# WindowsXp-Beta/nos

Hardware: AMD Instinct MI355X
Metric: aggregate GPU util % + schedulable fractional pods/node at 1/2/4/8 MI355X (higher is better)
Workload: dtype fp32

## Files before the change

### csrc/hip/gemm_f32h.hip

```cpp
#include <stdlib.h>

#include <type_traits>

#include "attn_d64_planes.h"
#include "common.h"
#include "epilogue.h"
#include "lds_pipe.h"
#include "split_f16.h"

namespace {

using nos::gelu_erf;
using nos::glds16;
using nos::wait_stages;

template <int E>
using EpiC = std::integral_constant<int, E>;

struct Batch {
  int nb = 1;
  long long a = 0, rinv = 0, w = 0, csc = 0, c = 0, r = 0, bias = 0;
};

constexpr int BK = 32;

__device__ __forceinline__ int swz(int row) { return (row >> 2) & 3; }

using nos::kvp::KvOut;

struct PlaneOut {
  unsigned short* p = nullptr;
  long long pplane = 0;
  int ldp = 0;
  float sc = 1.f;
};

struct LnIo {
  const float* x = nullptr;
  const float2* sin = nullptr;
  float2* sout = nullptr;
  int ldx = 0, nparts = 0, pw = 0, spart = 0;
  float eps = 0.f, sc = 1.f;
};

__device__ __forceinline__ void chan_merge(float& n, float& mean, float& m2, float nb, float mb, float m2b) {
  const float tot = n + nb;
  if (!(nb > 0.f)) return;
  const float d = mb - mean, f = nb / tot;
  mean = fmaf(d, f, mean);
  m2 += m2b + d * d * n * f;
  n = tot;
}

template <int BM, int BN, int WGM, int WGN, bool PERSIST, int RS = 2, int MODE = 0, bool BATCHED = false>
__global__ __launch_bounds__(64 * WGM * WGN, 2) void gemm_h3_kernel(
    const _Float16* __restrict__ Ap, int lda, long long aplane, const float* __restrict__ rinv, float rconst,
    const _Float16* __restrict__ Wp, int ldw, long long wplane, const float* __restrict__ csc,
    const float* __restrict__ bias, const float* __restrict__ R, int ldr0, float* __restrict__ C, int ldc0, int M,
    int N, int K, int epi, int tiles_m, int tiles_n, KvOut kv, PlaneOut po, Batch bt, LnIo ln) {
  constexpr int NW = WGM * WGN, MI = BM / (32 * WGM), NI = BN / (32 * WGN);
  static_assert(NW == 4 && MI >= 1 && NI >= 1, "4 waves");
  constexpr int ROWB = BK * 2, CH = ROWB / 16, RPP = 1024 / ROWB;
  static_assert(RS == 2 || RS == 3, "ring depth");
  constexpr int TA = 2 * BM * ROWB, STAGE = TA + 2 * BN * ROWB;
  constexpr int APW = TA / 1024 / NW, WPW = 2 * BN * ROWB / 1024 / NW;
  static_assert(APW * NW * 1024 == TA && WPW * NW * 1024 == 2 * BN * ROWB, "equal DMA count per wave");
  constexpr int LPS = APW + WPW;
  static_assert((RS - 2) * LPS < 64, "vmcnt range");
  static_assert(MODE == 0 || (BM == 128 && !BATCHED && (BN == 128 || BN == 64) && (RS == 2 || (MODE == 2 && RS == 3))),
                "the LayerNorm hand-off runs 128 x 128 or 128 x 64 tiles (the producer also on a 3-deep ring)");
  static_assert(MODE != 2 || BM * BN * 4 <= RS * STAGE, "the statistics tile fits the ring");
  extern __shared__ __attribute__((aligned(16))) unsigned char smem[];

  const int tid = threadIdx.x, wid = __builtin_amdgcn_readfirstlane(tid >> 6), lane = tid & 63;
  const int c0 = lane & 31, h0 = lane >> 5;
  const int wm = wid / WGN, wn = wid % WGN;
  const bool wide = (epi & EPI_WIDE) != 0;
  epi &= ~EPI_WIDE;
  const int ntiles1 = tiles_m * tiles_n, ntiles = BATCHED ? ntiles1 * bt.nb : ntiles1;
  const int nk = K / BK;
  nos::XcdChunk chunk;
  if constexpr (PERSIST) {
    chunk = nos::xcd_chunk(blockIdx.x, gridDim.x, ntiles);
  } else {
    chunk.first = nos::xcd_remap(blockIdx.x, ntiles);
    chunk.end = chunk.first + 1;
    chunk.step = 1;
  }
  for (int tt = chunk.first; tt < chunk.end; tt += chunk.step) {
    if (PERSIST && tt != chunk.first) __syncthreads();
    const int bb = BATCHED ? tt / ntiles1 : 0, t1 = BATCHED ? tt - bb * ntiles1 : tt;
    const int tm = t1 / tiles_n, tn = t1 - tm * tiles_n;
    const int m0 = tm * BM, n0 = tn * BN;
    const _Float16* __restrict__ Ab = BATCHED ? Ap + bb * bt.a : Ap;
    const _Float16* __restrict__ Wb = BATCHED ? Wp + bb * bt.w : Wp;
    const float* __restrict__ rinvb = BATCHED && rinv != nullptr ? rinv + bb * bt.rinv : rinv;
    const float* __restrict__ cscb = BATCHED ? csc + bb * bt.csc : csc;
    float* __restrict__ Cb = BATCHED && C != nullptr ? C + bb * bt.c : C;
    const float* __restrict__ Rb = BATCHED && R != nullptr ? R + bb * bt.r : R;
    const float* __restrict__ biasb = BATCHED && bias != nullptr ? bias + bb * bt.bias : bias;

    auto stage_a = [&](int k0, unsigned char* dst) {
#pragma unroll
      for (int i = 0; i < APW; ++i) {
        const int p = wid * APW + i;
        const int plane = p / (BM / RPP), rb = (p % (BM / RPP)) * RPP;
        const int row = rb + lane / CH;
        int g = m0 + row;
        g = g < M ? g : M - 1;
        glds16(Ab + plane * aplane + (long long)g * lda + k0 + (((lane % CH) ^ swz(row)) << 3),
               dst + plane * BM * ROWB + rb * ROWB);
      }
    };
    auto stage_w = [&](int k0, unsigned char* dst) {
#pragma unroll
      for (int i = 0; i < WPW; ++i) {
        const int p = wid * WPW + i;
        const int plane = p / (BN / RPP), rb = (p % (BN / RPP)) * RPP;
        const int row = rb + lane / CH;
        int g = n0 + row;
        g = g < N ? g : N - 1;
        glds16(Wb + plane * wplane + (long long)g * ldw + k0 + (((lane % CH) ^ swz(row)) << 3),
               dst + TA + plane * BN * ROWB + rb * ROWB);
      }
    };
    auto stage = [&](int k0, unsigned char* dst) {
      stage_a(k0, dst);
      stage_w(k0, dst);
    };

    f32x16_t acc[MI][NI];
#pragma unroll
    for (int i = 0; i < MI; ++i)
#pragma unroll
      for (int j = 0; j < NI; ++j)
#pragma unroll
        for (int r = 0; r < 16; ++r) acc[i][j][r] = 0.f;

    struct Frag {
      f16x8_t a[MI][2], w[NI][2];
    };
    auto load = [&](const unsigned char* base, int s, Frag& f) {
#pragma unroll
      for (int i = 0; i < MI; ++i) {
        const int row = wm * (BM / WGM) + i * 32 + c0;
#pragma unroll
        for (int p = 0; p < 2; ++p)
          f.a[i][p] = *reinterpret_cast<const f16x8_t*>(base + p * BM * ROWB + row * ROWB +
                                                        (((2 * s + h0) ^ swz(row)) << 4));
      }
#pragma unroll
      for (int j = 0; j < NI; ++j) {
        const int row = wn * (BN / WGN) + j * 32 + c0;
#pragma unroll
        for (int p = 0; p < 2; ++p)
          f.w[j][p] = *reinterpret_cast<const f16x8_t*>(base + TA + p * BN * ROWB + row * ROWB +
                                                        (((2 * s + h0) ^ swz(row)) << 4));
      }
    };
    auto mma = [&](const Frag& f) {
#pragma unroll
      for (int i = 0; i < MI; ++i)
#pragma unroll
        for (int j = 0; j < NI; ++j) acc[i][j] = nos::mma3h(f.a[i], f.w[j], acc[i][j]);
    };

    if constexpr (MODE == 1) {
    constexpr int AR = BM * 4 / (64 * NW);
    constexpr int RSTEP = 64 * NW / 4;
    const int q = tid & 3;
    float mul[AR], add[AR];
    const float* xr[AR];
#pragma unroll
    for (int i = 0; i < AR; ++i) {
      int g = m0 + (tid >> 2) + RSTEP * i;
      g = g < M ? g : M - 1;
      xr[i] = ln.x + (long long)g * ln.ldx + q * 8;
      const float2* st = ln.sin + (long long)g * ln.nparts;
      float n = 0.f, mean = 0.f, m2 = 0.f;
      for (int p = 0; p < ln.nparts; ++p) {
        const float2 v = st[p];
        const int nb = min(ln.pw, K - p * ln.pw);
        chan_merge(n, mean, m2, (float)nb, v.x, v.y);
      }
      mul[i] = rsqrtf(m2 / (float)K + ln.eps) * ln.sc;
      add[i] = -mean * mul[i];
    }
    float4 xa[AR][2];
    auto aload = [&](int k0) {
#pragma unroll
      for (int i = 0; i < AR; ++i) {
        xa[i][0] = *reinterpret_cast<const float4*>(xr[i] + k0);
        xa[i][1] = *reinterpret_cast<const float4*>(xr[i] + k0 + 4);
      }
    };
    auto awrite = [&](unsigned char* dst) {
#pragma unroll
      for (int i = 0; i < AR; ++i) {
        const int row = (tid >> 2) + RSTEP * i;
        const float4 u = xa[i][0], w = xa[i][1];
        f16x2_t h0, l0, h1, l1, h2, l2, h3, l3;
        nos::split2h(f32x2_t{fmaf(u.x, mul[i], add[i]), fmaf(u.y, mul[i], add[i])}, h0, l0);
        nos::split2h(f32x2_t{fmaf(u.z, mul[i], add[i]), fmaf(u.w, mul[i], add[i])}, h1, l1);
        nos::split2h(f32x2_t{fmaf(w.x, mul[i], add[i]), fmaf(w.y, mul[i], add[i])}, h2, l2);
        nos::split2h(f32x2_t{fmaf(w.z, mul[i], add[i]), fmaf(w.w, mul[i], add[i])}, h3, l3);
        const int off = row * ROWB + ((q ^ swz(row)) << 4);
        *reinterpret_cast<f16x8_t*>(dst + off) = f16x8_t{h0.x, h0.y, h1.x, h1.y, h2.x, h2.y, h3.x, h3.y};
        *reinterpret_cast<f16x8_t*>(dst + BM * ROWB + off) = f16x8_t{l0.x, l0.y, l1.x, l1.y, l2.x, l2.y, l3.x, l3.y};
      }
    };
    aload(0);
    stage_w(0, smem);
    asm volatile("s_waitcnt vmcnt(0)" ::: "memory");
    awrite(smem);
    if (nk > 1) {
      aload(BK);
      stage_w(BK, smem + STAGE);
    }
    asm volatile("s_waitcnt lgkmcnt(0)" ::: "memory");
    __builtin_amdgcn_s_barrier();
    Frag fa, fb;
    load(smem, 0, fa);
    for (int kt = 0; kt < nk; ++kt) {
      const unsigned char* cur = smem + (kt & 1) * STAGE;
      load(cur, 1, fb);
      mma(fa);
      __builtin_amdgcn_sched_barrier(0);
      if (kt + 1 < nk) {
        asm volatile("s_waitcnt vmcnt(0)" ::: "memory");
        awrite(smem + ((kt + 1) & 1) * STAGE);
      }
      __builtin_amdgcn_sched_barrier(0);
      mma(fb);
      __builtin_amdgcn_sched_barrier(0);
      if (kt + 1 < nk) {
        asm volatile("s_waitcnt lgkmcnt(0)" ::: "memory");
        __builtin_amdgcn_s_barrier();
        if (kt + 2 < nk) {
          aload((kt + 2) * BK);
          stage_w((kt + 2) * BK, smem + (kt & 1) * STAGE);
        }
        load(smem + ((kt + 1) & 1) * STAGE, 0, fa);
      }
      __builtin_amdgcn_sched_barrier(0);
    }
    } else if constexpr (RS == 2) {
    stage(0, smem);
    if (nk > 1) stage(BK, smem + STAGE);
    if (nk > 1) {
      asm volatile("s_waitcnt vmcnt(%0)" ::"n"(LPS) : "memory");
    } else {
      asm volatile("s_waitcnt vmcnt(0)" ::: "memory");
    }
    __builtin_amdgcn_s_barrier();
    Frag fa, fb;
    load(smem, 0, fa);
    for (int kt = 0; kt < nk; ++kt) {
      const unsigned char* cur = smem + (kt & 1) * STAGE;
      load(cur, 1, fb);
      mma(fa);
      __builtin_amdgcn_sched_barrier(0);
      if (kt + 1 < nk) {
        asm volatile("s_waitcnt vmcnt(0)" ::: "memory");
        asm volatile("s_waitcnt lgkmcnt(0)" ::: "memory");
        __builtin_amdgcn_s_barrier();
        if (kt + 2 < nk) stage((kt + 2) * BK, smem + (kt & 1) * STAGE);
        load(smem + ((kt + 1) & 1) * STAGE, 0, fa);
      }
      mma(fb);
      __builtin_amdgcn_sched_barrier(0);
    }
    } else {
#pragma unroll
    for (int q = 0; q < RS - 1; ++q)
      if (q < nk) stage(q * BK, smem + q * STAGE);
    for (int kt = 0; kt < nk; ++kt) {
      wait_stages<LPS>(min(RS - 2, nk - 1 - kt));
      asm volatile("s_waitcnt lgkmcnt(0)" ::: "memory");
      __builtin_amdgcn_s_barrier();
      if (kt + RS - 1 < nk) stage((kt + RS - 1) * BK, smem + ((kt + RS - 1) % RS) * STAGE);
      const unsigned char* cur = smem + (kt % RS) * STAGE;
      Frag f0, f1;
      load(cur, 0, f0);
      load(cur, 1, f1);
      mma(f0);
      mma(f1);
    }
    }
    __syncthreads();

    int c = c0, h = h0, ldc = ldc0, ldr = ldr0;
    asm volatile("" : "+v"(c), "+v"(h));
    asm volatile("" : "+s"(ldc), "+s"(ldr));
    float rsv[MI][16], rbv[MI][16];
    if (rinvb != nullptr) {
#pragma unroll
      for (int i = 0; i < MI; ++i)
#pragma unroll
        for (int r = 0; r < 16; ++r) {
          const int m = m0 + wm * (BM / WGM) + i * 32 + (r & 3) + 8 * (r >> 2) + 4 * h;
          rsv[i][r] = rinvb[m < M ? m : M - 1];
        }
    } else {
#pragma unroll
      for (int i = 0; i < MI; ++i)
#pragma unroll
        for (int r = 0; r < 16; ++r) rsv[i][r] = rconst;
    }
#pragma unroll
    for (int i = 0; i < MI; ++i)
#pragma unroll
      for (int r = 0; r < 16; ++r) {
        const int m = m0 + wm * (BM / WGM) + i * 32 + (r & 3) + 8 * (r >> 2) + 4 * h;
        rbv[i][r] = (BATCHED && (epi & EPI_BIAS_ROW)) ? biasb[m < M ? m : M - 1] : 0.f;
      }
    auto epilogue = [&](auto ec) -> bool {
      constexpr int E = decltype(ec)::value;
      auto has = [&](int f) -> bool {
        if constexpr (E < 0) return (epi & f) != 0;
        else return (E & f) != 0;
      };
      if constexpr (MODE == 2) {
// ... 146 lines not shown
              const int rl = wm * (BM / WGM) + i * 32 + (r & 3) + 8 * (r >> 2) + 4 * h;
              float v = fmaf(acc[i][j][r], rsv[i][r] * cs, p2 + rbv[i][r]);
              if (BATCHED && has(EPI_RESID_PRE)) v += Rt[(unsigned)(rl * ldr + cl)];
              if (has(EPI_GELU)) v = gelu_erf(v);
              if (has(EPI_RELU)) v = fmaxf(v, 0.f);
              if (has(EPI_RESID)) v += Rt[(unsigned)(rl * ldr + cl)];
              Ct[(unsigned)(rl * ldc + cl)] = v;
            }
          }
        }
        return true;
      }
      return false;
    };
    bool done = false;
    if constexpr (MODE == 1) {
      if (epi == EPI_BIAS) done = epilogue(EpiC<EPI_BIAS>{});
      else if (epi == (EPI_BIAS | EPI_GELU)) done = epilogue(EpiC<EPI_BIAS | EPI_GELU>{});
      else done = epilogue(EpiC<-1>{});
    } else if constexpr (MODE == 2) {
      if (epi == (EPI_BIAS | EPI_RESID)) done = epilogue(EpiC<EPI_BIAS | EPI_RESID>{});
      else if (epi == EPI_BIAS) done = epilogue(EpiC<EPI_BIAS>{});
      else done = epilogue(EpiC<-1>{});
    } else if constexpr (BATCHED) {
      done = epilogue(EpiC<-1>{});
    } else {
      switch (epi) {
        case EPI_BIAS: done = epilogue(EpiC<EPI_BIAS>{}); break;
        case EPI_BIAS | EPI_GELU: done = epilogue(EpiC<EPI_BIAS | EPI_GELU>{}); break;
        case EPI_BIAS | EPI_RESID: done = epilogue(EpiC<EPI_BIAS | EPI_RESID>{}); break;
        default: done = epilogue(EpiC<-1>{}); break;
      }
    }
    if (done) continue;
#pragma unroll
    for (int j = 0; j < NI; ++j) {
      const int n = n0 + wn * (BN / WGN) + j * 32 + c;
      const int nc = n < N ? n : N - 1;
      const float cs = cscb[nc];
      const float p2 = (epi & EPI_BIAS) ? biasb[nc] : 0.f;
#pragma unroll
      for (int i = 0; i < MI; ++i) {
#pragma unroll
        for (int r = 0; r < 16; ++r) {
          const int m = m0 + wm * (BM / WGM) + i * 32 + (r & 3) + 8 * (r >> 2) + 4 * h;
          float v = fmaf(acc[i][j][r], rsv[i][r] * cs, p2 + rbv[i][r]);
          if (BATCHED && (epi & EPI_RESID_PRE) && m < M && n < N) v += Rb[(long long)m * ldr + n];
          if ((epi & EPI_GELU)) v = gelu_erf(v);
          if ((epi & EPI_RELU)) v = fmaxf(v, 0.f);
          if (m < M && n < N) {
            if ((epi & EPI_RESID)) v += Rb[(long long)m * ldr + n];
            if (kv.kvs != nullptr && n >= kv.qcols) {
              const int t = (n - kv.qcols) >= kv.hd;
              const int col = n - kv.qcols - t * kv.hd;
              const int b = kv.S == M ? 0 : m / kv.S;
              const long long row = (long long)b * kv.skvp + (m - b * kv.S);
              const float x = v * kv.kvsc[t * (kv.hd >> 6) + (col >> 6)];
              const _Float16 h0 = (_Float16)x;
              const _Float16 h1 = (_Float16)(x - (float)h0);
              unsigned short* dst = kv.kvs + (row * nos::kvp::H3 + nos::kvp::H3 / 2 * t) * kv.hd + col;
              dst[0] = __builtin_bit_cast(unsigned short, h0);
              dst[kv.hd] = __builtin_bit_cast(unsigned short, h1);
            } else if (po.p != nullptr) {
              const float x = v * po.sc;
              const _Float16 h0 = (_Float16)x;
              const _Float16 h1 = (_Float16)(x - (float)h0);
              po.p[(long long)m * po.ldp + n] = __builtin_bit_cast(unsigned short, h0);
              po.p[po.pplane + (long long)m * po.ldp + n] = __builtin_bit_cast(unsigned short, h1);
            } else {
              Cb[(long long)m * ldc + n] = v;
            }
          }
        }
      }
    }
  }
}

bool g_wide_planes = [] {
  const char* e = getenv("NOS_AMD_H3_WIDE_PLANES");
  return e == nullptr || atoi(e) != 0;
}();

bool wide_planes_ok(const KvOut& kv, const PlaneOut& po) {
  if (!g_wide_planes) return false;
  if (po.p != nullptr)
    return !(((uintptr_t)po.p) & 15) && !(po.ldp % 8) && !(po.pplane % 8);
  if (kv.kvs != nullptr) return !(((uintptr_t)kv.kvs) & 15) && !(kv.hd % 8) && !(kv.qcols % 8);
  return false;
}

struct H3Call {
  const _Float16* a = nullptr;
  int lda = 0;
  long long aplane = 0;
  const float* rinv = nullptr;
  float rconst = 0.f;
  const _Float16* w = nullptr;
  int ldw = 0;
  long long wplane = 0;
  const float* csc = nullptr;
  const float* bias = nullptr;
  const float* R = nullptr;
  int ldr = 0;
  float* C = nullptr;
  int ldc = 0;
  int M = 0, N = 0, K = 0, epi = 0;
  KvOut kv;
  PlaneOut po;
  Batch bt;
  LnIo ln;
};

template <int BM, int BN, int WGM, int WGN, int RS = 2, bool BATCHED = false, int MODE = 0>
int launch_t(const H3Call& c, hipStream_t st) {
  const int tiles_m = (c.M + BM - 1) / BM, tiles_n = (c.N + BN - 1) / BN;
  const long long ntiles = (long long)tiles_m * tiles_n * c.bt.nb;
  if (ntiles > (1LL << 30)) return (int)hipErrorInvalidValue;
  const size_t lds = RS * (size_t)(2 * BM * BK * 2 + 2 * BN * BK * 2);
  constexpr int NT = 64 * WGM * WGN;
  const int epi = !BATCHED && wide_planes_ok(c.kv, c.po) ? c.epi | EPI_WIDE : c.epi;
  auto* plain = gemm_h3_kernel<BM, BN, WGM, WGN, false, RS, MODE, BATCHED>;
  decltype(plain) persistent = nullptr;
  if constexpr (!BATCHED) persistent = gemm_h3_kernel<BM, BN, WGM, WGN, true, RS, MODE, BATCHED>;
  return nos::launch_items(persistent, plain, NT, lds, ntiles, st, c.a, c.lda, c.aplane, c.rinv, c.rconst, c.w, c.ldw,
                           c.wplane, c.csc, c.bias, c.R, c.ldr, c.C, c.ldc, c.M, c.N, c.K, epi, tiles_m, tiles_n, c.kv,
                           c.po, c.bt, c.ln);
}

bool g_lds_epi = true;
int g_hot_ring = 2;
int g_hot_bn = 128;

template <int F4, int LPR = 64>
__global__ __launch_bounds__(256) void split_rows_h3_kernel(const float* __restrict__ A, int lda,
                                                            _Float16* __restrict__ P, int ldp, long long pplane,
                                                            float* __restrict__ rinv, int M, int K, int ln,
                                                            float eps, int eln) {
  typedef __attribute__((ext_vector_type(4))) _Float16 f16x4_t;
  constexpr int RPB = 256 / LPR;
  const int row = blockIdx.x * RPB + (int)(threadIdx.x / LPR);
  const int lane = threadIdx.x % LPR;
  if (row >= M) return;
  const float* a = A + (long long)row * lda;
  constexpr int NR = F4 > 0 ? F4 : 1;
  float4 v[NR];
  auto get = [&](int i, int k) -> float4 {
    if constexpr (F4 > 0) return v[i];
    return *reinterpret_cast<const float4*>(a + k);
  };
  const int nchunk = F4 > 0 ? F4 : (K + 4 * LPR - 1) / (4 * LPR);
  if constexpr (F4 > 0) {
#pragma unroll
    for (int i = 0; i < F4; ++i) {
// ... 151 lines not shown
  for (int o = 16; o > 0; o >>= 1) q += __shfl_xor(q, o, 64);
  if (lane == 0) out[row] = float2{mu, q};
}

}

NOS_API int nos_row_stats(const float* X, int ldx, void* stats, int M, int K, hipStream_t stream) {
  if (M <= 0 || K <= 0 || (K % 4) || (ldx % 4) || ldx < K || !X || !stats || (((uintptr_t)X) & 15) ||
      (((uintptr_t)stats) & 7))
    return (int)hipErrorInvalidValue;
  hipLaunchKernelGGL(row_stats_kernel, dim3((unsigned)((M + 7) / 8)), dim3(256), 0, stream, X, ldx,
                     static_cast<float2*>(stats), M, K);
  return (int)hipGetLastError();
}

NOS_API int nos_gemm_f32h3_set_lds_epilogue(int on) {
  g_lds_epi = on != 0;
  return 0;
}

NOS_API int nos_gemm_f32h3_set_hot_bn(int bn) {
  if (bn != 128 && bn != 64) return (int)hipErrorInvalidValue;
  g_hot_bn = bn;
  return 0;
}

NOS_API int nos_gemm_f32h3_hot_bn() { return g_hot_bn; }

NOS_API int nos_gemm_f32h3_set_hot_ring(int rs) {
  if (rs != 2 && rs != 3) return (int)hipErrorInvalidValue;
  g_hot_ring = rs;
  return 0;
}

NOS_API int nos_split_rows_h3(const float* A, int lda, void* P, int ldp, long long pplane, float* rinv, int M, int K,
                              int ln, float eps, int eln, hipStream_t stream) {
  if (M <= 0 || K <= 0 || (K % 4) || (lda % 4) || (ldp % 4) || ldp < K || pplane < (long long)M * ldp)
    return (int)hipErrorInvalidValue;
  if ((((uintptr_t)A) | ((uintptr_t)P)) & 15) return (int)hipErrorInvalidValue;
  if (eln < -126 || eln > 126 || ln < 0 || ln > 2) return (int)hipErrorInvalidValue;
  auto* p = static_cast<_Float16*>(P);
  const dim3 grid((unsigned)((M + 3) / 4)), blk(256);
  if (K <= 512) {
    const dim3 g2((unsigned)((M + 7) / 8));
    hipLaunchKernelGGL((split_rows_h3_kernel<4, 32>), g2, blk, 0, stream, A, lda, p, ldp, pplane, rinv, M, K, ln, eps,
                       eln);
  } else if (K <= 1024)
    hipLaunchKernelGGL(split_rows_h3_kernel<4>, grid, blk, 0, stream, A, lda, p, ldp, pplane, rinv, M, K, ln, eps, eln);
  else if (K <= 2048)
    hipLaunchKernelGGL(split_rows_h3_kernel<8>, grid, blk, 0, stream, A, lda, p, ldp, pplane, rinv, M, K, ln, eps, eln);
  else if (K <= 4096)
    hipLaunchKernelGGL(split_rows_h3_kernel<16>, grid, blk, 0, stream, A, lda, p, ldp, pplane, rinv, M, K, ln, eps,
                       eln);
  else
    hipLaunchKernelGGL(split_rows_h3_kernel<0>, grid, blk, 0, stream, A, lda, p, ldp, pplane, rinv, M, K, ln, eps, eln);
  return (int)hipGetLastError();
}

NOS_API int nos_split_cols_h3(const float* X, int ldx, long long bsx, int M, int K, int nb, void* P, int ldp,
                              long long pplane, float* rinv, float* work, hipStream_t stream) {
  const int Mp = (M + 31) / 32 * 32;
  if (M <= 0 || K <= 0 || nb <= 0 || ldx < K || (nb > 1 && bsx < (long long)(M - 1) * ldx + K) || ldp < Mp ||
      (ldp % 8) || pplane < (long long)nb * K * ldp || !X || !P || !rinv || !work || nb > 65535 ||
      (long long)(M + 63) / 64 > 65535)
    return (int)hipErrorInvalidValue;
  if ((((uintptr_t)P) & 15) || (pplane % 8)) return (int)hipErrorInvalidValue;
// ... 165 lines not shown
```

### csrc/hip/lds_pipe.h

```cpp
#pragma once
#include "common.h"

namespace nos {

__device__ __forceinline__ void glds16(const void* g, unsigned char* lds_wave_base) {
  const unsigned lds = __builtin_amdgcn_readfirstlane(
      (unsigned)(uintptr_t)(__attribute__((address_space(3))) unsigned char*)lds_wave_base);
  asm volatile("s_nop 0\n\tglobal_load_lds_dwordx4 %0, off" ::"v"(g), "{m0}"(lds) : "memory");
}

__device__ __forceinline__ void glds16_s(const void* sbase, unsigned voff, unsigned char* lds_wave_base) {
  const unsigned lds = __builtin_amdgcn_readfirstlane(
      (unsigned)(uintptr_t)(__attribute__((address_space(3))) unsigned char*)lds_wave_base);
  asm volatile("s_nop 0\n\tglobal_load_lds_dwordx4 %0, %1" ::"v"(voff), "s"(sbase), "{m0}"(lds) : "memory");
}

__device__ __forceinline__ void glds16_builtin(const void* g, unsigned char* lds_wave_base) {
  __builtin_amdgcn_global_load_lds(g, (__attribute__((address_space(3))) void*)lds_wave_base, 16, 0, 0);
}

__device__ __forceinline__ void dma_wait_publish() {
  asm volatile("s_waitcnt vmcnt(0)" ::: "memory");
  __syncthreads();
}

template <int LPS>
__device__ __forceinline__ void wait_stages(int n) {
  if (n <= 0)
    asm volatile("s_waitcnt vmcnt(0)" ::: "memory");
  else if (n == 1)
    asm volatile("s_waitcnt vmcnt(%0)" ::"n"(LPS) : "memory");
  else if (n == 2)
    asm volatile("s_waitcnt vmcnt(%0)" ::"n"(2 * LPS) : "memory");
  else
    asm volatile("s_waitcnt vmcnt(%0)" ::"n"(3 * LPS) : "memory");
}

}
```

### nos_amd/models/pod.py

```python
from __future__ import annotations

import argparse
import json
import os
import sys
import time
from pathlib import Path
from typing import Callable

import numpy as np

STATE_STARTING, STATE_READY, STATE_FAILED, STATE_DONE = 0.0, 1.0, 2.0, 3.0
_COLS = 4


class StatusBoard:

    def __init__(self, path: str | os.PathLike, pods: int | None = None):
        self.path = Path(path)
        if pods is not None:
            np.zeros((1 + pods, _COLS), dtype=np.float64).tofile(self.path)
        self.arr = np.memmap(self.path, dtype=np.float64, mode="r+")
        self.arr = self.arr.reshape(-1, _COLS)

# ... 34 lines not shown
    elif dtype == "bf16":
        from ..ops import _lib

        _lib.require_native_on_gpu()
        m = YolosDetector(cfg, backend="native")
        tdt = torch.bfloat16
    else:
        raise ValueError(f"dtype {dtype!r}")
    m.reset_parameters(seed)
    m = m.to(device, tdt).eval()
    x = make_demo_input(cfg, device=device, dtype=tdt, hw=hw if device == "cuda" else cfg.image_size, seed=seed)
    return m, x


def _die_with_parent() -> Callable[[], bool]:
    ppid0 = os.getppid()
    try:
        import ctypes
        import signal

        ctypes.CDLL(None, use_errno=True).prctl(1, int(signal.SIGTERM), 0, 0, 0)
    except Exception:
        pass
    return lambda: os.getppid() != ppid0


def kernel_config(memory_fraction: float | None, env: dict | None = None, cu_budget: int = 0) -> dict[str, str]:
    env = os.environ if env is None else env
    whole = memory_fraction is None or memory_fraction >= 0.99
    if cu_budget and not whole:
        gf = "latency"
    else:
        gf = "latency" if whole else "small"
    return {"gemm_bf16": env.get("NOS_AMD_GEMM_POLICY") or ("latency" if whole else "throughput"),
            "gemm_f32": env.get("NOS_AMD_GEMM_F32_POLICY") or gf,
            "attention_f32": env.get("NOS_AMD_ATTN_F32_VARIANT") or ("h3" if whole else "h3n"),
            "f32_math": env.get("NOS_AMD_F32_MATH") or "h3",
            "gemm_f32x6_tile": env.get("NOS_AMD_X6_TILE") or ("policy" if whole else "128x128"),
            "ln_handoff": env.get("NOS_AMD_LN_HANDOFF") or "on",
            "h3_epilogue": env.get("NOS_AMD_H3_EPILOGUE") or "lds",
            "h3_hot_ring": env.get("NOS_AMD_H3_HOT_RING") or "2",
            "h3_hot_bn": env.get("NOS_AMD_H3_HOT_BN") or "128"}


def slice_cu_budget(env: dict | None = None) -> int:
    env = os.environ if env is None else env
    if env.get("NOS_AMD_CU_BUDGET") is not None:
        return int(env["NOS_AMD_CU_BUDGET"])
    m = env.get("ROC_GLOBAL_CU_MASK")
    if not m:
        return 0
    try:
        return bin(int(m, 16)).count("1")
    except ValueError:
        return 0


class _ServerTenant:

    def __init__(self, client, keep_outputs: bool = False):
        self.client, self.keep_outputs, self.outputs = client, keep_outputs, ()

    def launch(self) -> None:
        if self.keep_outputs:
            self.outputs = self.client.infer(outputs=True)[0]
        else:
            self.client.infer()
# ... 172 lines not shown
```

### nos_amd/ops/__init__.py

```python
from __future__ import annotations

import math
from typing import NamedTuple

import torch
import torch.nn.functional as F

from . import _lib

EPI_BIAS, EPI_GELU, EPI_RESID, EPI_RELU = 1, 2, 4, 8


def _stream() -> int:
    return torch.cuda.current_stream().cuda_stream


def _ptr(t: torch.Tensor | None) -> int | None:
    return None if t is None else t.data_ptr()


def linear_ref(x, weight, bias=None, act=None, residual=None):
    y = x.float() @ weight.float().t()
    if bias is not None:
        y = y + bias.float()
# ... 330 lines not shown
def h3_planes_active(attention: bool = False) -> bool:
    return _F32_MATH == "h3" and (not attention or _ATTN_F32_VARIANT.startswith("h3"))


def set_f32_math(mode: str) -> None:
    global _F32_MATH
    if mode not in ("exact", "x6", "h3"):
        raise ValueError(f"f32 math must be 'exact', 'x6' or 'h3', got {mode!r}")
    _F32_MATH = mode


def f32_math() -> str:
    return _F32_MATH


def set_gemm_f32x6_tile(tile: str) -> None:
    names = {"policy": -1, "128x64": 3, "128x128": 5, "wide": 6, "256x128": 7}
    code = names[tile] if tile in names else int(tile)
    _lib.check(_lib.lib().nos_gemm_f32x6_set_tile(code), "nos_gemm_f32x6_set_tile")


def set_gemm_f32h3_lds_epilogue(on: bool) -> None:
    _lib.check(_lib.lib().nos_gemm_f32h3_set_lds_epilogue(int(bool(on))), "nos_gemm_f32h3_set_lds_epilogue")


def set_gemm_f32h3_hot_ring(stages: int) -> None:
    _lib.check(_lib.lib().nos_gemm_f32h3_set_hot_ring(int(stages)), "nos_gemm_f32h3_set_hot_ring")


def set_gemm_f32h3_hot_bn(bn: int) -> None:
    _lib.check(_lib.lib().nos_gemm_f32h3_set_hot_bn(int(bn)), "nos_gemm_f32h3_set_hot_bn")


def stats_pw() -> int:
    return int(_lib.lib().nos_gemm_f32h3_hot_bn())


def set_gemm_f32x6_pipeline(on: bool) -> None:
    _lib.check(_lib.lib().nos_gemm_f32x6_set_pipeline(int(bool(on))), "nos_gemm_f32x6_set_pipeline")


def split_bf16x3(t: torch.Tensor) -> torch.Tensor:
    t = t.float()
    p0 = t.to(torch.bfloat16)
    r = t - p0.float()
    p1 = r.to(torch.bfloat16)
    p2 = (r - p1.float()).to(torch.bfloat16)
    return torch.stack([p0, p1, p2]).contiguous()


@torch.no_grad()
def split_f32_weight(w: torch.Tensor) -> torch.Tensor:
    key = id(w)
    hit = _SPLIT_CACHE.get(key)
    if hit is not None:
        ref, ver, ptr, planes = hit
        if ref() is w and ver == w._version and ptr == w.data_ptr():
            return planes
    import weakref

    planes = split_bf16x3(w)
    _SPLIT_CACHE[key] = (weakref.ref(w, lambda _r, k=key: _SPLIT_CACHE.pop(k, None)), w._version, w.data_ptr(),
                         planes)
    return planes


# ... 20 lines not shown


def set_attention_f32_variant(variant: str) -> None:
    global _ATTN_F32_VARIANT
    x6 = {"x6": 0, "x6n": 1, "x6k1": 1, "x6k2": 2, "x6k3": 3, "x6k4": 4,
          "h3": 0, "h3n": 1, "h3k1": 1, "h3k2": 2, "h3k3": 3, "h3k4": 4}
    code = {"auto": 0, "w4k64": 1, "w4k64g2": 2, "w4k32": 3, "w2k64": 4, "w8k64": 5, "w4k32o4": 6,
            "w4k32g2": 7}.get(variant, 0)
    if variant not in x6 and code == 0 and variant != "auto":
        raise KeyError(variant)
    _lib.check(_lib.lib().nos_attn_f32_set_variant(code), "nos_attn_f32_set_variant")
    if variant in x6:
        _lib.check(_lib.lib().nos_attn_f32x6_set_kvsplit(x6[variant]), "nos_attn_f32x6_set_kvsplit")
    _ATTN_F32_VARIANT = variant


_ATTN_F32_VARIANT = "auto"


def attention_f32_variant() -> str:
    return _ATTN_F32_VARIANT


def apply_kernel_config(cfg: dict) -> None:
    set_gemm_policy(cfg["gemm_bf16"])
    set_gemm_f32_policy(cfg["gemm_f32"])
    set_attention_f32_variant(cfg["attention_f32"])
    set_f32_math(cfg["f32_math"])
    set_gemm_f32x6_tile(cfg["gemm_f32x6_tile"])
    set_ln_handoff(cfg.get("ln_handoff", "on") == "on")
    set_gemm_f32h3_lds_epilogue(cfg.get("h3_epilogue", "lds") == "lds")
    set_gemm_f32h3_hot_ring(int(cfg.get("h3_hot_ring", "2")))
    set_gemm_f32h3_hot_bn(int(cfg.get("h3_hot_bn", "128")))


@torch.no_grad()
def fold_layernorm(weight: torch.Tensor, bias: torch.Tensor | None, gamma: torch.Tensor, beta: torch.Tensor
                   ) -> tuple[torch.Tensor, torch.Tensor, torch.Tensor]:
    wg = (weight.float() * gamma.float()[None, :]).to(weight.dtype).contiguous()
    c1 = wg.float().sum(dim=1).contiguous()
    c2 = (weight.float() * beta.float()[None, :]).sum(dim=1)
    if bias is not None:
        c2 = c2 + bias.float()
    return wg, c1, c2.contiguous()


def linear_ln_ref(x, wg, c1, c2, act=None, eps=1e-12):
    xf = x.float()
    mu = xf.mean(-1, keepdim=True)
    var = xf.var(-1, unbiased=False, keepdim=True)
    y = ((xf @ wg.float().t()) - mu * c1) * torch.rsqrt(var + eps) + c2
    if act == "gelu":
        y = F.gelu(y)
    elif act == "relu":
        y = F.relu(y)
    return y.to(x.dtype)


def linear_ln(x: torch.Tensor, wg: torch.Tensor, c1: torch.Tensor, c2: torch.Tensor, act: str | None = None,
              eps: float = 1e-12, out: torch.Tensor | None = None, max_wg: int = 0,
              pre=None) -> torch.Tensor:
    if not x.is_cuda:
        return linear_ln_ref(x, wg, c1, c2, act, eps)
    K = x.shape[-1]
    N = wg.shape[0]
    x2 = x.reshape(-1, K)
# ... 294 lines not shown
```

### nos_amd/ops/_lib.py

```python
from __future__ import annotations

import ctypes
import os
import threading
from pathlib import Path

_LIB_PATH = Path(os.environ.get("NOS_AMD_HIP_LIB") or
                 Path(__file__).resolve().parent.parent / "_native" / "libnos_hip.so")
_lock = threading.Lock()
_lib: ctypes.CDLL | None = None
_err: str | None = None

c_int, c_ll, c_float, c_void_p, c_double = (ctypes.c_int, ctypes.c_longlong, ctypes.c_float,
                                            ctypes.c_void_p, ctypes.c_double)

_SIGS = {
    "nos_attn_fwd_d64": [c_void_p, c_void_p, c_void_p, c_void_p, c_int, c_int, c_int, c_int, c_int,
                         c_ll, c_int, c_ll, c_float, c_void_p],
    "nos_attn_fwd_f32_d64": [c_void_p, c_void_p, c_void_p, c_void_p, c_int, c_int, c_int, c_int, c_int,
                             c_ll, c_int, c_ll, c_float, c_void_p],
    "nos_attn_fwd_f32x6_d64": [c_void_p, c_void_p, c_void_p, c_void_p, c_int, c_int, c_int, c_int, c_int,
                               c_ll, c_int, c_ll, c_float, c_void_p, c_ll, c_void_p],
    "nos_attn_f32x6_workspace": [c_int, c_int, c_int, c_int],
    "nos_attn_fwd_f32x6_presplit_d64": [c_void_p, c_void_p, c_int, c_int, c_int, c_int, c_int, c_ll, c_int, c_ll,
# ... 111 lines not shown
                 c_int, c_int, c_int, c_float, c_void_p],
    "nos_gemv_partials": [c_void_p, c_ll, c_int, c_int, c_int, c_int, c_int, c_int, c_void_p, c_int, c_int, c_void_p,
                          c_void_p, c_int, c_void_p, c_int, c_int, c_int, c_int, c_int, c_void_p],
    "nos_gemv_q8": [c_void_p, c_int, c_void_p, c_int, c_void_p, c_void_p, c_void_p, c_void_p, c_int, c_void_p, c_int,
                    c_int, c_int, c_int, c_int, c_float, c_void_p],
    "nos_gemv_q8_partials": [c_void_p, c_ll, c_int, c_int, c_int, c_int, c_int, c_void_p, c_int, c_void_p, c_void_p,
                             c_void_p, c_int, c_void_p, c_int, c_int, c_int, c_int, c_int, c_void_p],
    "nos_dequant_q8": [c_void_p, c_int, c_void_p, c_void_p, c_int, c_int, c_int, c_void_p],
    "nos_lora_shrink": [c_void_p, c_int, c_void_p, c_ll, c_int, c_int, c_int, c_int, c_void_p, c_ll, c_int, c_void_p,
                        c_int, c_int, c_void_p, c_float, c_void_p, c_int, c_int, c_int, c_void_p],
    "nos_gemv_lora": [c_void_p, c_int, c_void_p, c_ll, c_int, c_int, c_int, c_int, c_void_p, c_int, c_void_p, c_void_p,
                      c_int, c_void_p, c_int, c_int, c_int, c_int, c_int, c_float, c_void_p, c_void_p, c_ll, c_int,
                      c_void_p, c_int, c_int, c_int, c_void_p],
    "nos_gemv_q8_lora": [c_void_p, c_int, c_void_p, c_ll, c_int, c_int, c_int, c_int, c_void_p, c_int, c_void_p,
                         c_void_p, c_void_p, c_void_p, c_int, c_void_p, c_int, c_int, c_int, c_int, c_int, c_float,
                         c_void_p, c_void_p, c_ll, c_int, c_void_p, c_int, c_int, c_int, c_void_p],
    "nos_moe_route": [c_void_p, c_int, c_void_p, c_int, c_void_p, c_float, c_void_p, c_void_p, c_int, c_int, c_int,
                      c_int, c_void_p],
    "nos_moe_glu": [c_void_p, c_int, c_void_p, c_void_p, c_ll, c_int, c_void_p, c_float, c_void_p, c_int, c_int, c_int,
                    c_int, c_int, c_void_p],
    "nos_moe_down": [c_void_p, c_void_p, c_void_p, c_void_p, c_ll, c_int, c_void_p, c_int, c_void_p, c_int, c_int,
                     c_int, c_int, c_int, c_int, c_void_p],
    "nos_attn_h3g_workspace": [c_int, c_int, c_int, c_int, c_int, c_int],
    "nos_gemm_f32h3_stats": [c_void_p, c_int, c_ll, c_void_p, c_float, c_void_p, c_int, c_ll, c_void_p, c_void_p,
                             c_void_p, c_int, c_void_p, c_int, c_int, c_int, c_int, c_int, c_void_p, c_void_p],
    "nos_gemm_f32h3_lna": [c_void_p, c_int, c_void_p, c_int, c_int, c_float, c_int, c_void_p, c_int, c_ll, c_void_p,
                           c_void_p, c_void_p, c_int, c_void_p, c_int, c_int, c_int, c_int, c_int, c_void_p, c_int,
                           c_int, c_void_p, c_void_p, c_int, c_ll, c_float, c_void_p],
    "nos_row_stats": [c_void_p, c_int, c_void_p, c_int, c_int, c_void_p],
    "nos_gemm_f32h3_set_lds_epilogue": [c_int],
    "nos_gemm_f32h3_set_hot_ring": [c_int],
    "nos_gemm_f32h3_set_hot_bn": [c_int],
    "nos_gemm_f32h3_hot_bn": [],
    "nos_attn_h3g_set_kvsplit": [c_int],
    "nos_attn_h3g": [c_void_p, c_int, c_ll, c_void_p, c_int, c_ll, c_void_p, c_int, c_ll, c_void_p, c_int, c_ll,
                     c_int, c_int, c_int, c_int, c_int, c_int, c_int, c_float, c_void_p, c_void_p, c_float, c_void_p,
                     c_ll, c_void_p],
    "nos_attn_h3g_lse": [c_void_p, c_int, c_ll, c_void_p, c_int, c_ll, c_void_p, c_int, c_ll, c_void_p, c_int, c_ll,
                         c_int, c_int, c_int, c_int, c_int, c_int, c_int, c_float, c_void_p, c_void_p, c_float,
                         c_void_p, c_ll, c_void_p, c_void_p],
    "nos_attn_h3g_bwd_workspace": [c_int, c_int, c_int, c_int, c_int, c_int],
    "nos_attn_h3g_bwd": [c_void_p, c_int, c_ll, c_void_p, c_int, c_ll, c_void_p, c_int, c_ll, c_void_p, c_int, c_ll,
                         c_void_p, c_int, c_ll, c_void_p, c_void_p, c_int, c_ll, c_void_p, c_int, c_ll, c_void_p, c_int,
                         c_ll, c_int, c_int, c_int, c_int, c_int, c_int, c_int, c_float, c_void_p, c_ll, c_void_p],
}


_RESTYPES = {"nos_attn_f32x6_workspace": c_ll, "nos_attn_h3g_workspace": c_ll, "nos_attn_decode_workspace": c_ll,
             "nos_attn_h3g_bwd_workspace": c_ll}


class NativeUnavailable(RuntimeError):
    pass


def lib_path() -> Path:
    return _LIB_PATH


def _load() -> ctypes.CDLL:
    import torch

    if not _LIB_PATH.exists():
        raise NativeUnavailable(
            f"{_LIB_PATH} missing: run `python -m nos_amd._native.build` (hipcc, gfx950)")
    L = ctypes.CDLL(str(_LIB_PATH), mode=ctypes.RTLD_GLOBAL)
# ... 53 lines not shown
```

Baseline: 28.00.

## Add L2 prefetch touches for K-stages and epilogue operands in f32h3 GEMM

```diff
diff --git a/csrc/hip/gemm_f32h.hip b/csrc/hip/gemm_f32h.hip
--- a/csrc/hip/gemm_f32h.hip
+++ b/csrc/hip/gemm_f32h.hip
@@ -16,6 +16,8 @@
 
 template <int E>
 using EpiC = std::integral_constant<int, E>;
+
+constexpr int EPI_L2K_SHIFT = 16, EPI_L2E_SHIFT = 20, EPI_API_MASK = 0xffff, L2_AHEAD_MAX = 8;
 
 struct Batch {
   int nb = 1;
@@ -51,6 +53,20 @@
   m2 += m2b + d * d * n * f;
   n = tot;
 }
+
+#ifdef NOS_H3_TILE_PHASES
+constexpr int PHASE_SLOTS = 1 << 15;
+__device__ unsigned long long g_phase_clk[PHASE_SLOTS][4];
+__device__ unsigned g_phase_next;
+#define NOS_H3_PHASE(i)                                                                     \
+  do {                                                                                      \
+    if (!PERSIST && tid == 0 && ph_slot < (unsigned)PHASE_SLOTS) g_phase_clk[ph_slot][i] = wall_clock64(); \
+  } while (0)
+#else
+#define NOS_H3_PHASE(i) \
+  do {                  \
+  } while (0)
+#endif
 
 template <int BM, int BN, int WGM, int WGN, bool PERSIST, int RS = 2, int MODE = 0, bool BATCHED = false>
 __global__ __launch_bounds__(64 * WGM * WGN, 2) void gemm_h3_kernel(
@@ -75,8 +91,14 @@
   const int tid = threadIdx.x, wid = __builtin_amdgcn_readfirstlane(tid >> 6), lane = tid & 63;
   const int c0 = lane & 31, h0 = lane >> 5;
   const int wm = wid / WGN, wn = wid % WGN;
+#ifdef NOS_H3_TILE_PHASES
+  unsigned ph_slot = PHASE_SLOTS;
+  if (!PERSIST && tid == 0) ph_slot = atomicAdd(&g_phase_next, 1u);
+#endif
+  NOS_H3_PHASE(0);
   const bool wide = (epi & EPI_WIDE) != 0;
-  epi &= ~EPI_WIDE;
+  const int l2k = (epi >> EPI_L2K_SHIFT) & 15, l2e = (epi >> EPI_L2E_SHIFT) & 15;
+  epi &= EPI_API_MASK & ~EPI_WIDE;
   const int ntiles1 = tiles_m * tiles_n, ntiles = BATCHED ? ntiles1 * bt.nb : ntiles1;
   const int nk = K / BK;
   nos::XcdChunk chunk;
@@ -129,6 +151,74 @@
       stage_w(k0, dst);
     };
 
+    constexpr int NT = 64 * NW;
+    constexpr int TKA = (2 * BM + NT - 1) / NT, TKW = (2 * BN + NT - 1) / NT, TK = TKA + TKW;
+    unsigned char* const sink = smem + RS * STAGE;
+    auto touch_stage = [&](int k0) {
+      int t = tid;
+      asm volatile("" : "+v"(t));
+#pragma unroll
+      for (int i = 0; i < TKA; ++i) {
+        const int idx = min(t + i * NT, 2 * BM - 1);
+        if constexpr (MODE == 1) {
+          const int g = min(m0 + (idx >> 1), M - 1);
+          nos::l2_touch(ln.x + (long long)g * ln.ldx + k0 + (idx & 1) * 16, sink);
+        } else {
+          const int plane = idx / BM, g = min(m0 + idx % BM, M - 1);
+          nos::l2_touch(Ab + plane * aplane + (long long)g * lda + k0, sink);
+        }
+      }
+#pragma unroll
+      for (int i = 0; i < TKW; ++i) {
+        const int idx = min(t + i * NT, 2 * BN - 1);
+        const int plane = idx / BN, g = min(n0 + idx % BN, N - 1);
+        nos::l2_touch(Wb + plane * wplane + (long long)g * ldw + k0, sink);
+      }
+    };
+    constexpr int TER = (BM * (BN / 16) + NT - 1) / NT;
+    static_assert(TK + 1 + TER <= 8, "touch instructions in flight behind a stage's DMAs");
+    auto touch_epi = [&]() -> int {
+      int t = tid;
+      asm volatile("" : "+v"(t));
+      const int j = t & 7;
+      const float* p = cscb + min(n0 + 16 * j, N - 1);
+      if (t < 8) {
+        if (rinvb != nullptr) p = rinvb + min(m0 + 16 * j, M - 1);
+      } else if (t >= 16 && t < 24) {
+        if (epi & EPI_BIAS) p = biasb + min(n0 + 16 * j, N - 1);
+      } else if (t == 24) {
+        if (kv.kvs != nullptr && n0 >= kv.qcols) p = kv.kvsc + ((n0 - kv.qcols) >> 6);
+      }
+      nos::l2_touch(p, sink);
+      if (!(epi & EPI_RESID)) return 1;
+#pragma unroll
+      for (int i = 0; i < TER; ++i) {
+        const int idx = min(t + i * NT, BM * (BN / 16) - 1);
+        const int m = min(m0 + idx / (BN / 16), M - 1), cc = n0 + 16 * (idx % (BN / 16));
+        nos::l2_touch(Rb + (long long)m * ldr0 + (cc < N ? cc : n0), sink);
+      }
+      return 1 + TER;
+    };
+    int pend = 0;
+    if (l2k > 0)
+      for (int s = 2; s < min(2 + l2k, nk); ++s) touch_stage(s * BK);
+    if (l2e > 0 && nk < l2e) touch_epi();
+    auto lookahead = [&](int kt) {
+      int n = 0;
+      if (l2k > 0 && kt + 2 + l2k < nk) {
+        touch_stage((kt + 2 + l2k) * BK);
+        n = TK;
+      }
+      if (l2e > 0 && kt == nk - l2e) n += touch_epi();
+      pend = n;
+    };
+    auto wait_dmas = [&](int behind) {
+      if (behind + pend == 0)
+        asm volatile("s_waitcnt vmcnt(0)" ::: "memory");
+      else
+        nos::wait_vm(behind + pend);
+    };
+
     f32x16_t acc[MI][NI];
 #pragma unroll
     for (int i = 0; i < MI; ++i)
@@ -171,20 +261,13 @@
     const int q = tid & 3;
     float mul[AR], add[AR];
     const float* xr[AR];
+    const float2* st[AR];
 #pragma unroll
     for (int i = 0; i < AR; ++i) {
       int g = m0 + (tid >> 2) + RSTEP * i;
       g = g < M ? g : M - 1;
       xr[i] = ln.x + (long long)g * ln.ldx + q * 8;
-      const float2* st = ln.sin + (long long)g * ln.nparts;
-      float n = 0.f, mean = 0.f, m2 = 0.f;
-      for (int p = 0; p < ln.nparts; ++p) {
-        const float2 v = st[p];
-        const int nb = min(ln.pw, K - p * ln.pw);
-        chan_merge(n, mean, m2, (float)nb, v.x, v.y);
-      }
-      mul[i] = rsqrtf(m2 / (float)K + ln.eps) * ln.sc;
-      add[i] = -mean * mul[i];
+      st[i] = ln.sin + (long long)g * ln.nparts;
     }
     float4 xa[AR][2];
     auto aload = [&](int k0) {
@@ -209,16 +292,38 @@
         *reinterpret_cast<f16x8_t*>(dst + BM * ROWB + off) = f16x8_t{l0.x, l0.y, l1.x, l1.y, l2.x, l2.y, l3.x, l3.y};
       }
     };
+    stage_w(0, smem);
+    if (nk > 1) stage_w(BK, smem + STAGE);
     aload(0);
-    stage_w(0, smem);
+    float sn[AR], smean[AR], sm2[AR];
+#pragma unroll
+    for (int i = 0; i < AR; ++i) sn[i] = smean[i] = sm2[i] = 0.f;
+    for (int p = 0; p < ln.nparts; p += 2) {
+      const int p1 = min(p + 1, ln.nparts - 1);
+      float2 v0[AR], v1[AR];
+#pragma unroll
+      for (int i = 0; i < AR; ++i) {
+        v0[i] = st[i][p];
+        v1[i] = st[i][p1];
+      }
+      const int nb0 = min(ln.pw, K - p * ln.pw), nb1 = p + 1 < ln.nparts ? min(ln.pw, K - (p + 1) * ln.pw) : 0;
+#pragma unroll
+      for (int i = 0; i < AR; ++i) {
+        chan_merge(sn[i], smean[i], sm2[i], (float)nb0, v0[i].x, v0[i].y);
+        chan_merge(sn[i], smean[i], sm2[i], (float)nb1, v1[i].x, v1[i].y);
+      }
+    }
+#pragma unroll
+    for (int i = 0; i < AR; ++i) {
+      mul[i] = rsqrtf(sm2[i] / (float)K + ln.eps) * ln.sc;
+      add[i] = -smean[i] * mul[i];
+    }
     asm volatile("s_waitcnt vmcnt(0)" ::: "memory");
     awrite(smem);
-    if (nk > 1) {
-      aload(BK);
-      stage_w(BK, smem + STAGE);
-    }
+    if (nk > 1) aload(BK);
     asm volatile("s_waitcnt lgkmcnt(0)" ::: "memory");
     __builtin_amdgcn_s_barrier();
+    NOS_H3_PHASE(1);
     Frag fa, fb;
     load(smem, 0, fa);
     for (int kt = 0; kt < nk; ++kt) {
@@ -242,6 +347,7 @@
         }
         load(smem + ((kt + 1) & 1) * STAGE, 0, fa);
       }
+      lookahead(kt);
       __builtin_amdgcn_sched_barrier(0);
     }
     } else if constexpr (RS == 2) {
@@ -253,6 +359,7 @@
       asm volatile("s_waitcnt vmcnt(0)" ::: "memory");
     }
     __builtin_amdgcn_s_barrier();
+    NOS_H3_PHASE(1);
     Frag fa, fb;
     load(smem, 0, fa);
     for (int kt = 0; kt < nk; ++kt) {
@@ -261,12 +368,13 @@
       mma(fa);
       __builtin_amdgcn_sched_barrier(0);
       if (kt + 1 < nk) {
-        asm volatile("s_waitcnt vmcnt(0)" ::: "memory");
+        wait_dmas(0);
         asm volatile("s_waitcnt lgkmcnt(0)" ::: "memory");
         __builtin_amdgcn_s_barrier();
         if (kt + 2 < nk) stage((kt + 2) * BK, smem + (kt & 1) * STAGE);
         load(smem + ((kt + 1) & 1) * STAGE, 0, fa);
       }
+      lookahead(kt);
       mma(fb);
       __builtin_amdgcn_sched_barrier(0);
     }
@@ -275,10 +383,12 @@
     for (int q = 0; q < RS - 1; ++q)
       if (q < nk) stage(q * BK, smem + q * STAGE);
     for (int kt = 0; kt < nk; ++kt) {
-      wait_stages<LPS>(min(RS - 2, nk - 1 - kt));
+      wait_dmas(min(RS - 2, nk - 1 - kt) * LPS);
       asm volatile("s_waitcnt lgkmcnt(0)" ::: "memory");
       __builtin_amdgcn_s_barrier();
+      if (kt == 0) NOS_H3_PHASE(1);
       if (kt + RS - 1 < nk) stage((kt + RS - 1) * BK, smem + ((kt + RS - 1) % RS) * STAGE);
+      lookahead(kt);
       const unsigned char* cur = smem + (kt % RS) * STAGE;
       Frag f0, f1;
       load(cur, 0, f0);
@@ -288,6 +398,7 @@
     }
     }
     __syncthreads();
+    NOS_H3_PHASE(2);
 
     int c = c0, h = h0, ldc = ldc0, ldr = ldr0;
     asm volatile("" : "+v"(c), "+v"(h));
@@ -500,7 +611,10 @@
         default: done = epilogue(EpiC<-1>{}); break;
       }
     }
-    if (done) continue;
+    if (done) {
+      NOS_H3_PHASE(3);
+      continue;
+    }
 #pragma unroll
     for (int j = 0; j < NI; ++j) {
       const int n = n0 + wn * (BN / WGN) + j * 32 + c;
@@ -542,6 +656,7 @@
         }
       }
     }
+    NOS_H3_PHASE(3);
   }
 }
 
@@ -549,6 +664,8 @@
   const char* e = getenv("NOS_AMD_H3_WIDE_PLANES");
   return e == nullptr || atoi(e) != 0;
 }();
+
+int g_l2_k = 0, g_l2_e = 2;
 
 bool wide_planes_ok(const KvOut& kv, const PlaneOut& po) {
   if (!g_wide_planes) return false;
@@ -585,9 +702,10 @@
   const int tiles_m = (c.M + BM - 1) / BM, tiles_n = (c.N + BN - 1) / BN;
   const long long ntiles = (long long)tiles_m * tiles_n * c.bt.nb;
   if (ntiles > (1LL << 30)) return (int)hipErrorInvalidValue;
-  const size_t lds = RS * (size_t)(2 * BM * BK * 2 + 2 * BN * BK * 2);
+  const size_t lds = RS * (size_t)(2 * BM * BK * 2 + 2 * BN * BK * 2) + nos::L2_SINK_BYTES;
   constexpr int NT = 64 * WGM * WGN;
-  const int epi = !BATCHED && wide_planes_ok(c.kv, c.po) ? c.epi | EPI_WIDE : c.epi;
+  int epi = (!BATCHED && wide_planes_ok(c.kv, c.po) ? c.epi | EPI_WIDE : c.epi) & EPI_API_MASK;
+  if (!BATCHED) epi |= (g_l2_k << EPI_L2K_SHIFT) | (g_l2_e << EPI_L2E_SHIFT);
   auto* plain = gemm_h3_kernel<BM, BN, WGM, WGN, false, RS, MODE, BATCHED>;
   decltype(plain) persistent = nullptr;
   if constexpr (!BATCHED) persistent = gemm_h3_kernel<BM, BN, WGM, WGN, true, RS, MODE, BATCHED>;
@@ -805,6 +923,30 @@
   g_hot_ring = rs;
   return 0;
 }
+
+NOS_API int nos_gemm_f32h3_set_l2_ahead(int k_stages, int epi_stages) {
+  if (k_stages < 0 || k_stages > L2_AHEAD_MAX || epi_stages < 0 || epi_stages > L2_AHEAD_MAX)
+    return (int)hipErrorInvalidValue;
+  g_l2_k = k_stages;
+  g_l2_e = epi_stages;
+  return 0;
+}
+
+NOS_API int nos_gemm_f32h3_l2_ahead() { return g_l2_k + 16 * g_l2_e; }
+
+#ifdef NOS_H3_TILE_PHASES
+NOS_API int nos_gemm_f32h3_tile_phases(unsigned long long* dst, int max_slots) {
+  unsigned n = 0, zero = 0;
+  if (hipDeviceSynchronize() != hipSuccess || hipMemcpyFromSymbol(&n, HIP_SYMBOL(g_phase_next), sizeof n) != hipSuccess)
+    return -1;
+  n = n < (unsigned)PHASE_SLOTS ? n : (unsigned)PHASE_SLOTS;
+  n = (int)n < max_slots ? n : (unsigned)(max_slots > 0 ? max_slots : 0);
+  if (n && hipMemcpyFromSymbol(dst, HIP_SYMBOL(g_phase_clk), (size_t)n * 4 * sizeof(unsigned long long)) != hipSuccess)
+    return -1;
+  if (hipMemcpyToSymbol(HIP_SYMBOL(g_phase_next), &zero, sizeof zero) != hipSuccess) return -1;
+  return (int)n;
+}
+#endif
 
 NOS_API int nos_split_rows_h3(const float* A, int lda, void* P, int ldp, long long pplane, float* rinv, int M, int K,
                               int ln, float eps, int eln, hipStream_t stream) {
diff --git a/csrc/hip/lds_pipe.h b/csrc/hip/lds_pipe.h
--- a/csrc/hip/lds_pipe.h
+++ b/csrc/hip/lds_pipe.h
@@ -19,6 +19,26 @@
   __builtin_amdgcn_global_load_lds(g, (__attribute__((address_space(3))) void*)lds_wave_base, 16, 0, 0);
 }
 
+constexpr int L2_SINK_BYTES = 256;
+__device__ __forceinline__ void l2_touch(const void* g, unsigned char* lds_sink) {
+  const unsigned lds = __builtin_amdgcn_readfirstlane(
+      (unsigned)(uintptr_t)(__attribute__((address_space(3))) unsigned char*)lds_sink);
+  asm volatile("s_nop 0\n\tglobal_load_lds_dword %0, off" ::"v"(g), "{m0}"(lds) : "memory");
+}
+
+__device__ __forceinline__ void wait_vm(int n) {
+#define NOS_WAIT_VM_CASE(i) \
+  case i: asm volatile("s_waitcnt vmcnt(" #i ")" ::: "memory"); break;
+  switch (n) {
+    NOS_WAIT_VM_CASE(0) NOS_WAIT_VM_CASE(1) NOS_WAIT_VM_CASE(2) NOS_WAIT_VM_CASE(3) NOS_WAIT_VM_CASE(4)
+    NOS_WAIT_VM_CASE(5) NOS_WAIT_VM_CASE(6) NOS_WAIT_VM_CASE(7) NOS_WAIT_VM_CASE(8) NOS_WAIT_VM_CASE(9)
+    NOS_WAIT_VM_CASE(10) NOS_WAIT_VM_CASE(11) NOS_WAIT_VM_CASE(12) NOS_WAIT_VM_CASE(13) NOS_WAIT_VM_CASE(14)
+    NOS_WAIT_VM_CASE(15)
+    default: asm volatile("s_waitcnt vmcnt(16)" ::: "memory"); break;
+  }
+#undef NOS_WAIT_VM_CASE
+}
+
 __device__ __forceinline__ void dma_wait_publish() {
   asm volatile("s_waitcnt vmcnt(0)" ::: "memory");
   __syncthreads();
diff --git a/nos_amd/models/pod.py b/nos_amd/models/pod.py
--- a/nos_amd/models/pod.py
+++ b/nos_amd/models/pod.py
@@ -90,7 +90,9 @@
         gf = "latency"
     else:
         gf = "latency" if whole else "small"
-    return {"gemm_bf16": env.get("NOS_AMD_GEMM_POLICY") or ("latency" if whole else "throughput"),
+    l2 = {"h3_l2_ahead": env["NOS_AMD_H3_L2_AHEAD"]} if env.get("NOS_AMD_H3_L2_AHEAD") else {}
+    return {**l2,
+            "gemm_bf16": env.get("NOS_AMD_GEMM_POLICY") or ("latency" if whole else "throughput"),
             "gemm_f32": env.get("NOS_AMD_GEMM_F32_POLICY") or gf,
             "attention_f32": env.get("NOS_AMD_ATTN_F32_VARIANT") or ("h3" if whole else "h3n"),
             "f32_math": env.get("NOS_AMD_F32_MATH") or "h3",
diff --git a/nos_amd/ops/__init__.py b/nos_amd/ops/__init__.py
--- a/nos_amd/ops/__init__.py
+++ b/nos_amd/ops/__init__.py
@@ -386,6 +386,15 @@
     _lib.check(_lib.lib().nos_gemm_f32h3_set_hot_bn(int(bn)), "nos_gemm_f32h3_set_hot_bn")
 
 
+def set_gemm_f32h3_l2_ahead(k_stages: int, epi_stages: int) -> None:
+    _lib.check(_lib.lib().nos_gemm_f32h3_set_l2_ahead(int(k_stages), int(epi_stages)), "nos_gemm_f32h3_set_l2_ahead")
+
+
+def gemm_f32h3_l2_ahead() -> tuple[int, int]:
+    v = int(_lib.lib().nos_gemm_f32h3_l2_ahead())
+    return v % 16, v // 16
+
+
 def stats_pw() -> int:
     return int(_lib.lib().nos_gemm_f32h3_hot_bn())
 
@@ -472,6 +481,9 @@
     set_gemm_f32h3_lds_epilogue(cfg.get("h3_epilogue", "lds") == "lds")
     set_gemm_f32h3_hot_ring(int(cfg.get("h3_hot_ring", "2")))
     set_gemm_f32h3_hot_bn(int(cfg.get("h3_hot_bn", "128")))
+    if "h3_l2_ahead" in cfg:
+        k, e = (int(v) for v in str(cfg["h3_l2_ahead"]).split(","))
+        set_gemm_f32h3_l2_ahead(k, e)
 
 
 @torch.no_grad()
diff --git a/nos_amd/ops/_lib.py b/nos_amd/ops/_lib.py
--- a/nos_amd/ops/_lib.py
+++ b/nos_amd/ops/_lib.py
@@ -167,6 +167,8 @@
     "nos_gemm_f32h3_set_hot_ring": [c_int],
     "nos_gemm_f32h3_set_hot_bn": [c_int],
     "nos_gemm_f32h3_hot_bn": [],
+    "nos_gemm_f32h3_set_l2_ahead": [c_int, c_int],
+    "nos_gemm_f32h3_l2_ahead": [],
     "nos_attn_h3g_set_kvsplit": [c_int],
     "nos_attn_h3g": [c_void_p, c_int, c_ll, c_void_p, c_int, c_ll, c_void_p, c_int, c_ll, c_void_p, c_int, c_ll,
                      c_int, c_int, c_int, c_int, c_int, c_int, c_int, c_float, c_void_p, c_void_p, c_float, c_void_p,
```

New measurement: 28.00. Within noise of the previous version (+0.0%).
